# sbi-dev/sbi

Measured on AMD Instinct MI355X. Metric: NPE train (theta,x)-pairs/sec, higher is better.
Workload: dtype f32; 1 GPU; BASELINE configs[1]: NPE + NSF theta-dim 10, x-dim 10, 100000 simulations (90 000-row training split resident in HBM), batch 65536 per GPU, synthetic linear-Gaussian; step = shuffled batch gather (device sampler) + fused NPE training step (pack, loss fwd+bwd, grad all-reduce, clip+Adam); parallelism=dp1, rccl_ranks=1

## Files before the change

sbi_amd/csrc/nsf_train_kernel.h:

```cpp
#pragma once
#include <hip/hip_runtime.h>
#include <stdlib.h>
#include <string.h>
#include "nsf_device.h"
#include "nsf_plan_layout.h"

#define TR_NW 4
#define TR_ROWS 64
#define TR_MAXCH 4
#define TR_GRID_MAX 256
#define TR_SA 68
#define TR_SB 68
#define TR_SLOT(PT) (16 * (PT) + 1)
#define TR_LDK_FAST 50
#ifndef TR_LA
#define TR_LA 2
#endif
#ifndef TR_SPLINE_PRIO
#define TR_SPLINE_PRIO 0
#endif
#ifndef TR_H_SPLIT
#define TR_H_SPLIT 0
#endif
#ifndef TR_PSTASH
#define TR_PSTASH 1
#endif
#ifndef TR_NO_S0
#define TR_NO_S0 1
#endif

struct TrainPlan {
  int SA, SB, SS;
  int o_A0, o_A1, o_B, o_Bs, o_cnt;
  int o_xs;
  int o_wave, w_total;
  int w_zs, w_gys, w_gzs;
  int DCHB, PTW;
  int nch[2];
  int PLP;
  int grid, ntiles;
  int lds_floats;
  int overlay;
  float* grad_x;
};

constexpr int build_train_layout(const NsfPlan& pl, TrainPlan* tp) {
  if (pl.D > 15 || pl.H > 64 || pl.NB > 2 || (pl.NB < 1 && !pl.ctx_mlp)) return SBI_AMD_E_UNSUPPORTED;
  const int d_id_max = pl.shape[0].d_id > pl.shape[1].d_id ? pl.shape[0].d_id : pl.shape[1].d_id;
  if (d_id_max + pl.C + 1 > 32 || pl.C + 1 > 32) return SBI_AMD_E_UNSUPPORTED;
  tp->DCHB = 4 / pl.PT;
  if (tp->DCHB < 1) return SBI_AMD_E_UNSUPPORTED;
  if (tp->DCHB > 2) tp->DCHB = 2;
  tp->PTW = 16 * pl.PT;
  for (int par = 0; par < 2; ++par) {
    tp->nch[par] = (pl.shape[par].d_tr + tp->DCHB - 1) / tp->DCHB;
    if (tp->nch[par] > TR_MAXCH) return SBI_AMD_E_UNSUPPORTED;
  }
  tp->SA = TR_SA;
// ... 44 lines not shown
  if (NSF_DBG_ABL(pl.ablate, 512) && tp->grid > 4) tp->grid = 4;
  return 0;
}

constexpr sbi_amd_nsf_config kNsfDefaultCfg = {10, 10, 50, 10, 5, 2, 3.0f, 1e-3f, 1e-3f, 1e-3f, 1e-3f};
constexpr NsfPlan nsf_make_static_plan() {
  NsfPlan p{};
  nsf_build_layout(&kNsfDefaultCfg, TR_NW, &p);
  return p;
}
constexpr NsfPlan kStaticPl = nsf_make_static_plan();
constexpr TrainPlan nsf_make_static_train() {
  TrainPlan t{};
  build_train_layout(kStaticPl, &t);
  return t;
}
constexpr TrainPlan kStaticTp = nsf_make_static_train();
static_assert(kStaticPl.n_params == 98025 && kStaticTp.overlay == 0 && kStaticTp.nch[0] == 3, "default NSF layout");

static bool plan_is_static_default(const NsfPlan& pl, const TrainPlan& tp) {
  NsfPlan a = pl;
  a.B = a.min_w = a.min_h = a.min_d = a.lu_eps = a.sqrt_h = a.inv_sqrt_h = 0.f;
  a.one_minus_kw = a.one_minus_kh = a.d_const = a.log_z = 0.f;
  a.ablate = 0;
  const NsfPlan b = kStaticPl;
  if (memcmp(&a, &b, sizeof(NsfPlan)) != 0) return false;
  TrainPlan c = tp;
  c.grid = c.ntiles = 0;
  c.grad_x = nullptr;
  const TrainPlan d = kStaticTp;
  return memcmp(&c, &d, sizeof(TrainPlan)) == 0 && NSF_DBG_ABL(pl.ablate, 0x40000) == 0;
}

__device__ __forceinline__ void stage_D(float* __restrict__ st, int SA, int row, const LaneId& id,
                                        const f4 (&v)[NSF_HT], bool relu) {
#pragma unroll
  for (int mt = 0; mt < NSF_HT; ++mt)
#pragma unroll
    for (int r = 0; r < 4; ++r) {
      float a = v[mt][r];
      st[row * SA + 16 * mt + 4 * r + id.g] = relu ? fmaxf(a, 0.f) : a;
    }
}

__device__ __forceinline__ int il_col(int c) { return 4 * (c & 15) + (c >> 4); }
__device__ __forceinline__ void stage_DB(float* __restrict__ st, int SB, int row, const LaneId& id,
                                         const f4 (&v)[NSF_HT], bool relu) {
  static_assert(NSF_HT == 4, "one float4 per register row");
#pragma unroll
  for (int r = 0; r < 4; ++r) {
    f4 w = {v[0][r], v[1][r], v[2][r], v[3][r]};
    if (relu) w = {fmaxf(w[0], 0.f), fmaxf(w[1], 0.f), fmaxf(w[2], 0.f), fmaxf(w[3], 0.f)};
    *(f4*)(st + row * SB + 4 * (4 * r + id.g)) = w;
  }
}

__device__ __forceinline__ constexpr int dw_krow(int s) { return 16 * (s >> 2) + (s & 3); }

template <int NT, int SA, int SB, bool IL = false>
__device__ __forceinline__ void dw_gemm(const float* __restrict__ Ast, const float* __restrict__ Bst,
                                        int acol0, int bcol0, const LaneId& id, f4 (&acc)[NT], int nt_on = NT,
                                        int abl = 0, f4* accb = nullptr) {
  if (abl & 1) return;
  const float ones_b = id.j == 0 ? 1.f : 0.f;
  constexpr int KS = TR_ROWS / 4, LA = NT >= 3 ? TR_LA : 2 * TR_LA;
  const float* ap = Ast + 4 * id.g * SA + acol0 + id.j;
  const float* bp = IL ? Bst + 4 * id.g * SB + 4 * id.j + (bcol0 >> 4) : Bst + 4 * id.g * SB + bcol0 + id.j;
  float a[LA + 1], b[LA + 1][NT];
  auto load_b = [&](int u, int s) {
    if (IL && NT == 4) {
      const f4 w = *(const f4*)(bp + dw_krow(s) * SB);
#pragma unroll
      for (int nt = 0; nt < NT; ++nt) b[u][nt] = w[nt];
    } else {
#pragma unroll
      for (int nt = 0; nt < NT; ++nt) b[u][nt] = bp[dw_krow(s) * SB + (IL ? nt : 16 * nt)];
    }
  };
#pragma unroll
  for (int u = 0; u < LA; ++u) {
    a[u] = ap[dw_krow(u) * SA];
    load_b(u, u);
  }
#pragma unroll
  for (int s = 0; s < KS; ++s) {
    if (s + LA < KS) {
      a[(s + LA) % (LA + 1)] = ap[dw_krow(s + LA) * SA];
      load_b((s + LA) % (LA + 1), s + LA);
    }
    __builtin_amdgcn_sched_barrier(0);
#pragma unroll
    for (int nt = 0; nt < NT; ++nt)
      if (NT == 1 || nt < nt_on) acc[nt] = MFMA16(a[s % (LA + 1)], b[s % (LA + 1)][nt], acc[nt]);
    if (accb) *accb = MFMA16(a[s % (LA + 1)], ones_b, *accb);
    __builtin_amdgcn_sched_barrier(0);
  }
}

template <int NT, int SA>
__device__ __forceinline__ void dw_gemm_rs(const float* __restrict__ Ast, const float* __restrict__ Bst, int SBr,
                                           int acol0, int bcol0, const LaneId& id, f4 (&acc)[NT], int nt_on = NT,
                                           int abl = 0) {
  if (abl & 1) return;
  constexpr int KS = TR_ROWS / 4, LA = NT >= 4 ? TR_LA : 2 * TR_LA;
  const float* ap = Ast + 4 * id.g * SA + acol0 + id.j;
  const float* bp = Bst + 4 * id.g * SBr + bcol0 + id.j;
  float a[LA + 1], b[LA + 1][NT];
#pragma unroll
  for (int u = 0; u < LA; ++u) {
    a[u] = ap[dw_krow(u) * SA];
#pragma unroll
    for (int nt = 0; nt < NT; ++nt) b[u][nt] = bp[dw_krow(u) * SBr + 16 * nt];
  }
#pragma unroll
  for (int s = 0; s < KS; ++s) {
    if (s + LA < KS) {
      a[(s + LA) % (LA + 1)] = ap[dw_krow(s + LA) * SA];
#pragma unroll
      for (int nt = 0; nt < NT; ++nt) b[(s + LA) % (LA + 1)][nt] = bp[dw_krow(s + LA) * SBr + 16 * nt];
    }
    __builtin_amdgcn_sched_barrier(0);
#pragma unroll
    for (int nt = 0; nt < NT; ++nt)
      if (NT == 1 || nt < nt_on) acc[nt] = MFMA16(a[s % (LA + 1)], b[s % (LA + 1)][nt], acc[nt]);
    __builtin_amdgcn_sched_barrier(0);
  }
}

#define MFMA4(a, b, c) __builtin_amdgcn_mfma_f32_4x4x1f32((a), (b), (c), 0, 0, 0)
constexpr int TR_THIN_C0 = 48;
static_assert(kStaticPl.H == TR_THIN_C0 + 2 && kStaticPl.KSH == 13 && kStaticPl.NB == 2,
              "thin remainder: the static layout's hidden width leaves 2 real features (+ bias column) in tile 3");

template <int SA, int SB>
__device__ __forceinline__ void dw_thin(const float* __restrict__ Ast, const float* __restrict__ Bst, const LaneId& id,
                                        f4& accM, f4& accN) {
  const int l = id.lane;
  const float* aM = Ast + TR_THIN_C0 + (l & 3);
  const float* aN = Ast + l;
  const float* bM = Bst + il_col(l);
  const float* bN = Bst + il_col(TR_THIN_C0 + (l & 3));
  constexpr int KS = TR_ROWS / 4;
  float v[2][4][4];
  auto load = [&](int u, int s) {
#pragma unroll
    for (int g = 0; g < 4; ++g) {
      const int r = dw_krow(s) + 4 * g;
      v[u][g][0] = aM[r * SA];
      v[u][g][1] = bM[r * SB];
      v[u][g][2] = aN[r * SA];
      v[u][g][3] = bN[r * SB];
    }
  };
  load(0, 0);
#pragma unroll
  for (int s = 0; s < KS; ++s) {
    if (s + 1 < KS) load((s + 1) & 1, s + 1);
    __builtin_amdgcn_sched_barrier(0);
#pragma unroll
    for (int g = 0; g < 4; ++g) {
      accM = MFMA4(v[s & 1][g][0], v[s & 1][g][1], accM);
      accN = MFMA4(v[s & 1][g][2], v[s & 1][g][3], accN);
    }
    __builtin_amdgcn_sched_barrier(0);
  }
}
template <bool THIN>
__device__ __forceinline__ void dw_hidden(const float* __restrict__ Ast, const float* __restrict__ Bst, int gw,
                                          const LaneId& id, f4 (&acc)[4], int abl) {
  if constexpr (THIN) {
    if (abl & 1) return;
    if (gw == TR_NW - 1) dw_thin<TR_SA, TR_SB>(Ast, Bst, id, acc[0], acc[1]);
    else dw_gemm<3, TR_SA, TR_SB, true>(Ast, Bst, 16 * gw, 0, id, *reinterpret_cast<f4(*)[3]>(&acc[0]));
  } else {
    dw_gemm<4, TR_SA, TR_SB, true>(Ast, Bst, 16 * gw, 0, id, acc, 4, abl, nullptr);
  }
}

__device__ __forceinline__ void load_D(const float* __restrict__ st, int SA, int row, const LaneId& id,
                                       f4 (&v)[NSF_HT]) {
#pragma unroll
  for (int mt = 0; mt < NSF_HT; ++mt)
#pragma unroll
    for (int r = 0; r < 4; ++r) v[mt][r] = st[row * SA + 16 * mt + 4 * r + id.g];
}

__device__ __forceinline__ void grad_wave_sync(int* cnt, int target, int lane) {
  __builtin_amdgcn_fence(__ATOMIC_RELEASE, "workgroup");
  if (lane == 0) __hip_atomic_fetch_add(cnt, 1, __ATOMIC_RELAXED, __HIP_MEMORY_SCOPE_WORKGROUP);
  while (__hip_atomic_load(cnt, __ATOMIC_RELAXED, __HIP_MEMORY_SCOPE_WORKGROUP) < target) __builtin_amdgcn_s_sleep(1);
  __builtin_amdgcn_fence(__ATOMIC_ACQUIRE, "workgroup");
}

template <int KS, int MT, int LDK>
__device__ __forceinline__ void gemm_T_breg_ldk(const float* __restrict__ lds, const LinDesc& L, const LaneId& id,
                                                const f4 (&gb)[NSF_HT], f4 (&acc)[MT]) {
  const int ldk = LDK ? LDK : L.ldk;
  const float* base[MT];
#pragma unroll
  for (int mt = 0; mt < MT; ++mt) {
    const int f = 16 * mt + id.iperm;
    base[mt] = lds + L.l_w + id.g * ldk + (f < L.in ? f : 0);
  }
  const int kstride = 4 * ldk;
  constexpr int NP = (KS + 1) / 2;
  float a[2][2][MT];
#pragma unroll
  for (int u = 0; u < 2; ++u)
#pragma unroll
    for (int mt = 0; mt < MT; ++mt) a[0][u][mt] = u < KS ? base[mt][u * kstride] : 0.f;
#pragma unroll
  for (int p = 0; p < NP; ++p) {
    if (p + 1 < NP) {
#pragma unroll
      for (int u = 0; u < 2; ++u)
#pragma unroll
        for (int mt = 0; mt < MT; ++mt)
// ... 249 lines not shown
      }
#pragma unroll
      for (int p = 0; p < NP; ++p) {
        if (p + 1 < NP) {
#pragma unroll
          for (int u = 0; u < 2; ++u) {
            bb[(p + 1) & 1][u] = brow[4 * (2 * p + 2 + u)];
#pragma unroll
            for (int mt = 0; mt < NSF_HT; ++mt) a[(p + 1) & 1][u][mt] = wcol[mt][(2 * p + 2 + u) * kstride];
          }
        }
        __builtin_amdgcn_sched_barrier(0);
#pragma unroll
        for (int u = 0; u < 2; ++u)
#pragma unroll
          for (int mt = 0; mt < NSF_HT; ++mt) gh[mt] = MFMA16(a[p & 1][u][mt], bb[p & 1][u], gh[mt]);
        __builtin_amdgcn_sched_barrier(0);
      }
    }
  }
#pragma unroll
  for (int mt = 0; mt < NSF_HT; ++mt)
#pragma unroll
    for (int r = 0; r < 4; ++r) gh[mt][r] = (16 * mt + 4 * r + id.g < LF.in) ? gh[mt][r] : 0.f;
}
template <int PT>
__device__ __forceinline__ void wft_chunk(const float* __restrict__ lds, const LinDesc& LF, const NsfPlan& pl,
                                          const ShapeDesc& S, const LaneId& id, const float* __restrict__ Arow,
                                          int SA, int d0, f4 (&gh)[NSF_HT]) {
  if (LF.ldk == TR_LDK_FAST) wft_chunk_ldk<PT, TR_LDK_FAST>(lds, LF, pl, S, id, Arow, SA, d0, gh);
  else wft_chunk_ldk<PT, 0>(lds, LF, pl, S, id, Arow, SA, d0, gh);
}

__device__ __forceinline__ void write_tile(float* __restrict__ part, const LinDesc& L, int out0, int nt,
                                           const LaneId& id, const f4& acc) {
#pragma unroll
  for (int r = 0; r < 4; ++r) {
    const int out = out0 + 4 * id.g + r;
    const int in = 16 * nt + id.j;
    if (out < L.out) {
      if (in < L.in) part[L.g_w + out * L.in + in] = acc[r];
      else if (in == L.in) part[L.g_b + out] = acc[r];
    }
  }
}
__device__ __forceinline__ void write_thin(float* __restrict__ part, const LinDesc& L, const LaneId& id, const f4& accM,
                                           const f4& accN) {
  const int l = id.lane;
#pragma unroll
  for (int m = 0; m < 4; ++m) {
    const int outM = TR_THIN_C0 + m, inM = l;
    if (outM < L.out) {
      if (inM < L.in) part[L.g_w + outM * L.in + inM] = accM[m];
      else if (inM == L.in) part[L.g_b + outM] = accM[m];
    }
    const int outN = 4 * (l >> 2) + m, inN = TR_THIN_C0 + (l & 3);
    if (l < TR_THIN_C0 && outN < L.out) {
      if (inN < L.in) part[L.g_w + outN * L.in + inN] = accN[m];
      else if (inN == L.in) part[L.g_b + outN] = accN[m];
    }
  }
}
__device__ __forceinline__ void write_bias(float* __restrict__ part, const LinDesc& L, int out0, const LaneId& id,
                                           const f4& accb) {
  if (id.j != 0) return;
#pragma unroll
  for (int r = 0; r < 4; ++r) {
    const int out = out0 + 4 * id.g + r;
    if (out < L.out) part[L.g_b + out] = accb[r];
  }
}

__device__ __forceinline__ constexpr int cm_reps(const NsfPlan& pl) { return pl.ctx_reps; }
struct BwdIo {
  int t_hi, t_lo;
  const float* packed;
  const float* zstats;
  const float* stash;
  const float* x;
  const float* noise;
  float* gz[2];
  const float* row_w;
  float uni_w;
  long long n, x_rows;
  float* partial;
  float* grad_theta;
  const float* astash;
  const float* pstash;
  long long* dbg;
};
template <int K, int KSH, int NBT, int NCH, int NTW, bool HB, int SP = 0>
__global__ void __launch_bounds__(128 * TR_NW, HB ? 1 : 2)
nsf_bwd_layer_kernel(const NsfPlan pl_, const TrainPlan tp_, const BwdIo io) {
// ... 2 lines not shown
  const float* __restrict__ x = io.x;
  const float* __restrict__ row_w = io.row_w;
  const float uni_w = io.uni_w;
  const long long n = io.n, x_rows = io.x_rows;
  float* __restrict__ partial = io.partial;
  float* __restrict__ grad_theta = io.grad_theta;
  const float* __restrict__ astash = io.astash;
  long long* __restrict__ dbg = io.dbg;
  const NsfPlan& pl = SP != 0 ? kStaticPl : pl_;
  const TrainPlan& tp = SP != 0 ? kStaticTp : tp_;
#ifdef NSF_DEBUG
  const int dbg_tile_sel = pl_.ablate & 128;
#define NSF_ABL(bit) (pl_.ablate & (bit))
#define NSF_ABLV (pl_.ablate)
#define TS(i) do { if (dbg && t == 0 && blockIdx.x == 0 && (threadIdx.x & 63) == 0 && tile == (int)(blockIdx.x + (dbg_tile_sel ? gridDim.x : 0))) \
    dbg[(threadIdx.x >> 6) * 64 + (i)] = (long long)__builtin_readcyclecounter(); } while (0)
#else
#define NSF_ABL(bit) 0
#define NSF_ABLV 0
#define TS(i) do { } while (0)
#endif
  constexpr int PT = (3 * K - 1 + 15) / 16;
  constexpr int DCHB = (4 / PT) > 2 ? 2 : (4 / PT);
  extern __shared__ __attribute__((aligned(16))) float lds[];
  const int tid = threadIdx.x;
  const int wave = tid >> 6;
  const LaneId id = make_lane();
  constexpr bool cm = (NBT == 0);
  constexpr int NB = cm ? 1 : NBT;
  const int SLOTS = nsf_ast_slots(pl);
  const int reps = cm_reps(pl);
  const int D = pl.D, C = pl.C;
  constexpr int SA = TR_SA, SB = TR_SB;
  const int SS = tp.SS;
  float* Bt = lds + tp.o_B;
  float* Bs = lds + tp.o_Bs;
  const float* x_mean = zstats + 2 * D;
  const float* x_std = x_mean + C;

  if (NSF_ABL(256)) {
    for (int i = tid; i < tp.lds_floats; i += blockDim.x) lds[i] = __builtin_nanf("");
    __syncthreads();
  }
  const bool ov = tp.overlay != 0;
  if (!ov) stage_layer(lds, packed + (long long)io.t_hi * pl.img_floats, pl.lds_w_train_floats, tid, blockDim.x);
  if (tid == 0) *(int*)(lds + tp.o_cnt) = 0;
  if (tid < 32) {
    lds[tp.o_xs + tid] = tid < C ? x_mean[tid] : 0.f;
    lds[tp.o_xs + 32 + tid] = tid < C ? 1.f / x_std[tid] : 1.f;
  }
  const float* xs = lds + tp.o_xs;
  const int ntc = (C + 1 + 15) / 16;
  const f4 zero4 = {0.f, 0.f, 0.f, 0.f};
  const bool multi = (int)(blockIdx.x + gridDim.x) < tp_.ntiles;
#define BWD_T_VARS                                                                                                  \
  const int par = cm ? 0 : (t & 1);                                                                                 \
  const ShapeDesc& S = pl.shape[(SP != 0 || cm) ? 0 : par];                                                         \
  const bool is_last = (t == pl.T - 1);                                                                             \
  const float* img = packed + (long long)t * pl.img_floats;                                                         \
  const int F0 = ov ? S.final_off : 0;                                                                              \
  const float* ldsF = lds - F0;                                                                                     \
  const LinDesc& L0 = S.lin[0];                                                                                     \
  const LinDesc& LF = S.lin[S.fin];                                                                                 \
  const int nch = tp.nch[(SP != 0 || cm) ? 0 : par];                                                                \
  const int nt0 = (S.in0 + 1 + 15) / 16;                               \
                     \
// ... 4 lines not shown
  if (wave < TR_NW) {
    float* sc = lds + tp.o_wave + wave * tp.w_total;
    float* zs = sc + tp.w_zs;
    float* gys = sc + tp.w_gys;
    float* gzs = sc + tp.w_gzs;
    const int arow0 = 16 * wave;
    for (int i = id.lane; i < tp.w_total; i += 64) sc[i] = 0.f;
    const LaneId id0 = id;
    float zv[4], gv[4], xv[8], wv;
    auto fetch_inputs = [&](int t_, int tile_, const LaneId& id) {
      const long long row_ = (long long)tile_ * TR_ROWS + arow0 + id.j;
      const long long rs = row_ < n ? row_ : 0;
      const long long xr = (x_rows == n) ? rs : (x_rows == 1 ? 0 : rs % x_rows);
      const float* z_in = io.stash + (long long)t_ * n * D;
      const float* gz_up = (t_ == pl.T - 1) ? io.noise : io.gz[(t_ + 1) & 1];
      const int d_id_ = pl.shape[(SP != 0 || cm) ? 0 : (t_ & 1)].d_id;
#pragma unroll
      for (int u = 0; u < 4; ++u) {
        const int d = id.g + 4 * u;
        const int dc = d < D ? d : 0;
        zv[u] = z_in[rs * D + dc];
        gv[u] = __hip_atomic_load(gz_up + rs * D + dc, __ATOMIC_RELAXED, __HIP_MEMORY_SCOPE_AGENT);
      }
#pragma unroll
      for (int u = 0; u < 8; ++u) {
        const int c = id.g + 4 * u - d_id_;
        xv[u] = x[xr * C + ((c >= 0 && c < C) ? c : 0)];
      }
      wv = row_w ? row_w[rs] : uni_w;
    };
    for (int t = io.t_hi; t >= io.t_lo; --t) {
    BWD_T_VARS
    LaneId id = id0;
    asm volatile("" : "+v"(id.lane), "+v"(id.j), "+v"(id.g), "+v"(id.iperm));
    float* __restrict__ gz_dn = io.gz[t & 1];
    if (t == io.t_hi || !multi) fetch_inputs(t, blockIdx.x, id);
    for (int tile = blockIdx.x; tile < tp_.ntiles; tile += gridDim.x) {
      LaneId id = id0;
      asm volatile("" : "+v"(id.j), "+v"(id.g), "+v"(id.iperm));
      const long long row = (long long)tile * TR_ROWS + arow0 + id.j;
      const bool valid = row < n;
      const float wn = valid ? wv : 0.f;
      const float gld = -wn;
      const int trow = arow0 + id.j;
      const bool need_s0 = !TR_NO_S0 || ov || tile == (int)blockIdx.x;
      if (need_s0) __syncthreads();
      if (ov) {
        stage_layer(lds, img + F0, pl.lds_w_train_floats - F0, tid, blockDim.x);
        __syncthreads();
      }
      TS(0);
      float gzr[4];
      {
#pragma unroll
        for (int u = 0; u < 4; ++u) {
          const int d = id.g + 4 * u;
          const float gz = (valid && d < D) ? gv[u] : 0.f;
          gzr[u] = is_last ? wn * gz : gz;
          if (d < D) {
            zs[id.j * pl.ZW + d] = valid ? zv[u] : 0.f;
            gzs[id.j * pl.ZW + d] = gzr[u];
          }
        }
        wave_lds_fence();
#pragma unroll
        for (int u = 0; u < 8; ++u) {
          const int k = id.g + 4 * u;
          const int c = k - S.d_id;
          const int cc = (c >= 0 && c < C) ? c : 0;
          const int zd = 2 * k + (1 - par);
          const float zid = zs[id.j * pl.ZW + (zd < D ? zd : 0)];
          const float ctx = ((valid ? xv[u] : 0.f) - xs[cc]) * xs[32 + cc];
          float v = (k == S.in0) ? 1.f : 0.f;
          v = (c >= 0 && c < C) ? ctx : v;
          v = (k < S.d_id) ? zid : v;
          if (k < SS) Bs[trow * SS + k] = v;
        }
        for (int k = 32 + id.g; k < SS; k += 4) Bs[trow * SS + k] = 0.f;
      }
      float gus_r[4] = {0.f, 0.f, 0.f, 0.f};
      if (cm) {
        for (int k = id.g; k < D; k += 4) gys[id.j * pl.ZW + k] = gzs[id.j * pl.ZW + k];
      } else if (!(NSF_ABL(64))) {
        const float* Lm = ldsF + S.l_L;
        const float* Um = ldsF + S.l_U;
        f4 gu = zero4, gy = zero4;
        float al[4], bz[4], au[4];
#pragma unroll
        for (int s4 = 0; s4 < 4; ++s4) {
          al[s4] = Lm[(4 * s4 + id.g) * 16 + id.j];
          bz[s4] = gzr[s4];
          au[s4] = Um[(4 * id.g + s4) * 16 + id.j];
        }
#pragma unroll
        for (int s4 = 0; s4 < 4; ++s4) gu = MFMA16(al[s4], bz[s4], gu);
#pragma unroll
        for (int s4 = 0; s4 < 4; ++s4) gy = MFMA16(au[s4], gu[s4], gy);
#pragma unroll
        for (int ii = 0; ii < 4; ++ii) {
          gus_r[ii] = gu[ii];
          if (4 * id.g + ii < D) gys[id.j * pl.ZW + 4 * id.g + ii] = gy[ii];
        }
      }
      wave_lds_fence();
      const long long nt16 = (n + 15) / 16;
      const long long wt16 = (long long)tile * TR_NW + wave < nt16 ? (long long)tile * TR_NW + wave : nt16 - 1;
      const float* ast = astash + (((long long)t * nt16 + wt16) * SLOTS) * 1024 +
                         4 * id.lane;
      TS(1);
      __syncthreads();
      TS(2);

      f4 bt1[NSF_HT], bt2[NSF_HT], bsg[NSF_HT];
      f4 hpre[cm ? 2 : 1][NSF_HT];
      if (TR_SPLINE_PRIO) __builtin_amdgcn_s_setprio(TR_SPLINE_PRIO);
      for (int c = 0; c < nch; ++c) {
        const int d0 = c * DCHB;
        const int slot = id.g & 1, part = id.g >> 1;
        const int dd = d0 + slot;
        float* pp = lds + ((c & 1) ? tp.o_A1 : tp.o_A0) + trow * SA + slot * TR_SLOT(PT);
        if (slot < DCHB) {
          if (dd < S.d_tr && !(NSF_ABL(4))) {
            const int zi = id.j * pl.ZW + 2 * dd + par;
            float yv, gxv;
            rq_spline_pair_bwd<K>(pp, tp.PTW, zs[zi], gys[zi], gld, pl_, part, yv, gxv);
            if (part == 0) {
              zs[zi] = yv;
              gys[zi] = gxv;
            }
          } else if (part == 0) {
            for (int k = 0; k < tp.PTW; ++k) pp[k] = 0.f;
          }
        }
        TS(3 + c);
        __syncthreads();
      }
      if (TR_SPLINE_PRIO) __builtin_amdgcn_s_setprio(0);
      if (cm) {
        ast_load<KSH>(ast, reps > 0 ? reps - 1 : 0, hpre[0]);
        if (reps > 0) ast_load<KSH>(ast, reps, hpre[1]);
      } else {
        ast_load<KSH>(ast, 2 + 4 * (NB - 1), bt2);
        ast_load<KSH>(ast, 3 + 4 * (NB - 1), bsg);
        ast_load<KSH>(ast, 1 + 4 * (NB - 1), bt1);
      }
      float us_r[4] = {0.f, 0.f, 0.f, 0.f};
      if (!cm && !(NSF_ABL(64))) {
        const float* Um = ldsF + S.l_U;
        float au[4], by[4];
#pragma unroll
        for (int s4 = 0; s4 < 4; ++s4) {
          au[s4] = Um[id.j * 16 + 4 * s4 + id.g];
          by[s4] = zs[id.j * pl.ZW + 4 * s4 + id.g];
        }
        f4 uv = zero4;
#pragma unroll
        for (int s4 = 0; s4 < 4; ++s4) uv = MFMA16(au[s4], by[s4], uv);
#pragma unroll
        for (int ii = 0; ii < 4; ++ii) us_r[ii] = uv[ii];
      }
      {
        const int nxt = tile + (int)gridDim.x;
        const bool more = nxt < tp_.ntiles, hop = !more && multi && t > io.t_lo;
        fetch_inputs(hop ? t - 1 : t, more ? nxt : (hop ? (int)blockIdx.x : tile), id);
      }
      TS(8);
      __syncthreads();
      if (ov) {
        stage_layer(lds, img, S.final_off, tid, blockDim.x);
        __syncthreads();
      }
      TS(9);
      const bool hsplit = TR_H_SPLIT && !cm && !ov;
      f4 gh[NSF_HT];
      load_D(lds + o_AX, SA, trow, id, gh);
      wave_lds_fence();
      const bool want_gx = tp_.grad_x != nullptr;
      float* gx_row = want_gx ? tp_.grad_x + (valid ? row : 0) * C : nullptr;

      if (cm) {
        f4 ga[NSF_HT], gb[NSF_HT];
        for (int i = reps; i >= 1; --i) {
          if (i < reps) {
            ast_load<KSH>(ast, i - 1, hpre[0]);
            ast_load<KSH>(ast, i, hpre[1]);
            __syncthreads();
          }
#pragma unroll
          for (int mt = 0; mt < NSF_HT; ++mt)
#pragma unroll
            for (int r = 0; r < 4; ++r) ga[mt][r] = hpre[1][mt][r] > 0.f ? gh[mt][r] : 0.f;
          stage_D(lds + o_AY, SA, trow, id, ga, false);
          stage_DB(Bt, SB, trow, id, hpre[0], true);
          if (!HB && id.g == 0) Bt[trow * SB + il_col(pl.H)] = 1.f;
          __syncthreads();
#pragma unroll
          for (int mt = 0; mt < NSF_HT; ++mt) gb[mt] = zero4;
          gemm_T_breg<KSH, NSF_HT>(lds, S.lin[1], id, ga, gb, NSF_ABLV);
#pragma unroll
          for (int mt = 0; mt < NSF_HT; ++mt) gh[mt] = gb[mt];
        }
#pragma unroll
        for (int mt = 0; mt < NSF_HT; ++mt)
#pragma unroll
          for (int r = 0; r < 4; ++r) gh[mt][r] = hpre[0][mt][r] > 0.f ? gh[mt][r] : 0.f;
      } else {
#pragma unroll
        for (int b = NB - 1; b >= 0; --b) {
          f4 ga[NSF_HT], gb[NSF_HT];
          {
            f4 gc[NSF_HT];
#pragma unroll
            for (int mt = 0; mt < NSF_HT; ++mt)
#pragma unroll
              for (int r = 0; r < 4; ++r) {
                const float sgm = bsg[mt][r];
                ga[mt][r] = gh[mt][r] * sgm;
                gc[mt][r] = gh[mt][r] * bt2[mt][r] * sgm * (1.f - sgm);
              }
            stage_D(lds + o_AX, SA, trow, id, gc, false);
            if (want_gx)
              ctx_grad_update<KSH>(lds, S.lin[1 + 3 * b], id, gc, 0, C, xs, gx_row, valid, is_last && b == NB - 1);
            if (hsplit && b == NB - 1) {
              TS(50);
              __syncthreads();
              TS(51);
            }
            stage_D(lds + o_AY, SA, trow, id, ga, false);
          }
          stage_DB(Bt, SB, trow, id, bt1, true);
          if (!HB && id.g == 0) Bt[trow * SB + il_col(pl.H)] = 1.f;
          ast_load<KSH>(ast, 4 * b, hpre[0]);
          if (b > 0) {
            ast_load<KSH>(ast, 2 + 4 * (b - 1), bt2);
            ast_load<KSH>(ast, 3 + 4 * (b - 1), bsg);
          }
          TS(20 + 8 * b);
          __syncthreads();
          TS(21 + 8 * b);
#pragma unroll
          for (int mt = 0; mt < NSF_HT; ++mt) gb[mt] = zero4;
          gemm_T_breg<KSH, NSF_HT>(lds, S.lin[3 + 3 * b], id, ga, gb, NSF_ABLV);
#pragma unroll
          for (int mt = 0; mt < NSF_HT; ++mt)
#pragma unroll
            for (int r = 0; r < 4; ++r) ga[mt][r] = bt1[mt][r] > 0.f ? gb[mt][r] : 0.f;
          if (b > 0) ast_load<KSH>(ast, 1 + 4 * (b - 1), bt1);
          TS(22 + 8 * b);
          __syncthreads();
          TS(23 + 8 * b);
          stage_D(lds + o_AY, SA, trow, id, ga, false);
          stage_DB(Bt, SB, trow, id, hpre[0], true);
          if (!HB && id.g == 0) Bt[trow * SB + il_col(pl.H)] = 1.f;
          __syncthreads();
          TS(24 + 8 * b);
#pragma unroll
          for (int mt = 0; mt < NSF_HT; ++mt) gb[mt] = zero4;
          gemm_T_breg<KSH, NSF_HT>(lds, S.lin[2 + 3 * b], id, ga, gb, NSF_ABLV);
#pragma unroll
          for (int mt = 0; mt < NSF_HT; ++mt)
#pragma unroll
            for (int r = 0; r < 4; ++r) gh[mt][r] += hpre[0][mt][r] > 0.f ? gb[mt][r] : 0.f;
          TS(25 + 8 * b);
          if (b > 0) __syncthreads();
        }
      }

      stage_D(lds + o_AX, SA, trow, id, gh, false);
      TS(40);
      __syncthreads();
      TS(41);
      {
        f4 gin[1];
        gin[0] = zero4;
        gemm_T_breg<KSH, 1>(lds, L0, id, gh, gin, NSF_ABLV);
#pragma unroll
        for (int r = 0; r < 4; ++r) {
          const int k = 4 * r + id.g;
          if (k < S.d_id) gys[id.j * pl.ZW + 2 * k + (1 - par)] += gin[0][r];
        }
      }
      if (want_gx) ctx_grad_update<KSH>(lds, L0, id, gh, S.d_id, C, xs, gx_row, valid, is_last && cm);
      if (!cm) {
        float* Ay = lds + o_AY + trow * SA;
#pragma unroll
        for (int ii = 0; ii < 4; ++ii) {
          const int k = 4 * id.g + ii;
          const int o = id.j * pl.ZW + k;
          Ay[k] = k < D ? gus_r[ii] : (k == D ? gld : 0.f);
          Ay[16 + k] = k < D ? gzs[o] : 0.f;
          Bt[trow * SB + il_col(k)] = k < D ? zs[o] : (k == D ? 1.f : 0.f);
          Bt[trow * SB + il_col(16 + k)] = k < D ? us_r[ii] : (k == D ? 1.f : 0.f);
        }
      }
      TS(42);
      __syncthreads();
      for (int d = id.g; d < D; d += 4) {
        if (valid) {
          const float g = gys[id.j * pl.ZW + d];
          if (t > 0) gz_dn[row * D + d] = g;
          else if (grad_theta) grad_theta[row * D + d] = g * zstats[D + d];
        }
      }
      TS(43);
    }
    if (t > io.t_lo && !ov) stage_layer(lds, packed + (long long)(t - 1) * pl.img_floats, pl.lds_w_train_floats, tid, 64 * TR_NW);
    }

  } else {
    const int gw = wave - TR_NW;
    int* cnt = (int*)(lds + tp.o_cnt);
    int sync_target = 0;
    const LaneId id0 = id;
    f4 hl[NSF_HT];
    auto fetch_hl = [&](int t_, int tile_) {
      const long long nt16 = (n + 15) / 16;
      const long long wt16 = (long long)tile_ * TR_NW + gw < nt16 ? (long long)tile_ * TR_NW + gw : nt16 - 1;
      const float* ast = astash + (((long long)t_ * nt16 + wt16) * SLOTS) * 1024 +
                         4 * id0.lane;
      ast_load<KSH>(ast, cm ? reps : 4 * NB, hl);
    };
    constexpr bool use_pst = TR_PSTASH != 0;
    f4 pq[DCHB][PT];
    auto pq_load = [&](int t_, int tile_, int c_) {
      const long long nt16 = (n + 15) / 16;
      const long long wt16 = (long long)tile_ * TR_NW + gw < nt16 ? (long long)tile_ * TR_NW + gw : nt16 - 1;
      const float* pstw = io.pstash + ((long long)t_ * nt16 + wt16) * nsf_pst_tile_floats(pl) + 4 * id0.lane;
      const int d_tr_ = pl.shape[(SP != 0 || cm) ? 0 : (t_ & 1)].d_tr;
#pragma unroll
      for (int sl = 0; sl < DCHB; ++sl) {
        const int dd = c_ * DCHB + sl;
#pragma unroll
        for (int pt = 0; pt < PT; ++pt) pq[sl][pt] = pst_load<PT>(pstw, dd < d_tr_ ? dd : d_tr_ - 1, pt);
      }
    };
    auto pq_store = [&](float* __restrict__ arow, const LaneId& id, int c_, int d_tr_) {
#pragma unroll
      for (int sl = 0; sl < DCHB; ++sl)
        if (c_ * DCHB + sl < d_tr_) {
#pragma unroll
          for (int pt = 0; pt < PT; ++pt)
#pragma unroll
            for (int r = 0; r < 4; ++r) arow[id.j * SA + sl * TR_SLOT(PT) + 16 * pt + 4 * r + id.g] = pq[sl][pt][r];
        }
    };
    fetch_hl(io.t_hi, blockIdx.x);
    if (use_pst) pq_load(io.t_hi, blockIdx.x, 0);
    for (int t = io.t_hi; t >= io.t_lo; --t) {
    BWD_T_VARS
    LaneId id = id0;
    asm volatile("" : "+v"(id.lane), "+v"(id.j), "+v"(id.g), "+v"(id.iperm));
    f4 acc0[NTW], accC[NB][NTW], acc1[NB][4], acc2[NB][4], accF[NCH][4], accLU[1];
    f4 acc1b[HB ? NB : 1], acc2b[HB ? NB : 1], accFb[HB ? NCH : 1];
  #pragma unroll
    for (int i = 0; i < (HB ? NB : 1); ++i) { acc1b[i] = zero4; acc2b[i] = zero4; }
  #pragma unroll
    for (int i = 0; i < (HB ? NCH : 1); ++i) accFb[i] = zero4;
  #pragma unroll
    for (int i = 0; i < NTW; ++i) acc0[i] = zero4;
  #pragma unroll
    for (int b = 0; b < NB; ++b) {
  #pragma unroll
      for (int i = 0; i < NTW; ++i) accC[b][i] = zero4;
  #pragma unroll
      for (int i = 0; i < 4; ++i) { acc1[b][i] = zero4; acc2[b][i] = zero4; }
    }
  #pragma unroll
    for (int c = 0; c < NCH; ++c)
  #pragma unroll
      for (int i = 0; i < 4; ++i) accF[c][i] = zero4;
    accLU[0] = zero4;

    for (int tile = blockIdx.x; tile < tp_.ntiles; tile += gridDim.x) {
      LaneId id = id0;
      asm volatile("" : "+v"(id.j), "+v"(id.g), "+v"(id.iperm));
      const int trow = 16 * gw + id.j;
      const bool more_tiles = tile + (int)gridDim.x < tp_.ntiles;
      const int t_nxt = more_tiles ? t : (t > io.t_lo ? t - 1 : t);
      const int tile_nxt = more_tiles ? tile + (int)gridDim.x : (t > io.t_lo ? (int)blockIdx.x : tile);
      const bool need_s0 = !TR_NO_S0 || ov || tile == (int)blockIdx.x;
      if (need_s0) __syncthreads();
      else { sync_target += 4; grad_wave_sync(cnt, sync_target, id.lane); }
      if (ov) {
        stage_layer(lds, img + F0, pl.lds_w_train_floats - F0, tid, blockDim.x);
        __syncthreads();
      }
      TS(0);
      stage_DB(Bt, SB, trow, id, hl, false);
      if (!HB && id.g == 0) Bt[trow * SB + il_col(pl.H)] = 1.f;
      if (use_pst) {
        pq_store(lds + tp.o_A0 + 16 * gw * SA, id, 0, S.d_tr);
        if (1 < nch) pq_load(t, tile, 1);
      } else if (!(NSF_ABL(32))) final_layer_chunk_T<PT, KSH>(ldsF, lds + tp.o_A0 + 16 * gw * SA, pl, tp, S, id, hl, 0);
      f4 gh[NSF_HT];
  #pragma unroll
      for (int mt = 0; mt < NSF_HT; ++mt) gh[mt] = zero4;
      TS(1);
      __syncthreads();
      TS(2);
  #pragma unroll
      for (int k = 0; k <= NCH; ++k) {
        if (k <= nch) {
          if (k >= 1) {
            const int oa = ((k - 1) & 1) ? tp.o_A1 : tp.o_A0;
            const bool hsplit = TR_H_SPLIT && !cm && !ov;
            if (hsplit && k == nch) {
              if (!(NSF_ABL(2))) wft_chunk<PT>(ldsF, LF, pl, S, id, lds + oa + 16 * gw * SA, SA, (k - 1) * DCHB, gh);
              stage_D(lds + o_AX, SA, trow, id, gh, false);
              TS(9);
              __syncthreads();
            }
            if (!HB && DCHB == 2 && k == nch && (S.d_tr & 1)) {
              f4 (&af)[4] = accF[k - 1 < NCH ? k - 1 : 0];
              f4 part[PT < 3 ? PT : 1];
#pragma unroll
              for (int i = 0; i < (PT < 3 ? PT : 1); ++i) part[i] = af[i];
              dw_gemm<(PT < 3 ? PT : 1), TR_SA, TR_SB, true>(lds + oa, Bt, 16 * (gw % PT), 16 * PT * (gw / PT), id, part,
                                                             PT < 3 ? PT : 1, NSF_ABLV, nullptr);
#pragma unroll
              for (int i = 0; i < (PT < 3 ? PT : 1); ++i) af[i] = part[i];
            } else
            dw_gemm<4, TR_SA, TR_SB, true>(lds + oa, Bt, 16 * gw + (gw / PT < DCHB ? gw / PT : 0), 0, id,
                                           accF[k - 1 < NCH ? k - 1 : 0], 4, NSF_ABLV,
                                           HB ? &accFb[k - 1 < NCH ? k - 1 : 0] : nullptr);
            TS(13 + k);
            if (!(hsplit && k == nch) && !(NSF_ABL(2)))
              wft_chunk<PT>(ldsF, LF, pl, S, id, lds + oa + 16 * gw * SA, SA, (k - 1) * DCHB, gh);
          }
          TS(3 + 2 * k);
          if (k + 1 < nch) {
            if (k >= 1) { sync_target += 4; grad_wave_sync(cnt, sync_target, id.lane); }
            TS(17 + k);
            if (use_pst) {
              pq_store(lds + (((k + 1) & 1) ? tp.o_A1 : tp.o_A0) + 16 * gw * SA, id, k + 1, S.d_tr);
              if (k + 2 < nch) pq_load(t, tile, k + 2);
            } else if (!(NSF_ABL(32)))
              final_layer_chunk_T<PT, KSH>(ldsF, lds + (((k + 1) & 1) ? tp.o_A1 : tp.o_A0) + 16 * gw * SA, pl, tp, S, id,
                                           hl, (k + 1) * DCHB);
          }
          if (k == nch && !(TR_H_SPLIT && !cm && !ov)) stage_D(lds + o_AX, SA, trow, id, gh, false);
          TS(4 + 2 * k);
          __syncthreads();
          if (ov && k == nch) {
            stage_layer(lds, img, S.final_off, tid, blockDim.x);
            __syncthreads();
          }
        }
      }
      if (cm) {
        for (int i = reps; i >= 1; --i) {
          if (i < reps) __syncthreads();
          __syncthreads();
          dw_gemm<4, TR_SA, TR_SB, true>(lds + o_AY, Bt, 16 * gw, 0, id, acc1[0], 4, NSF_ABLV, HB ? &acc1b[0] : nullptr);
        }
      } else {
  #pragma unroll
        for (int b = NB - 1; b >= 0; --b) {
          __syncthreads();
          TS(21 + 8 * b);
          if constexpr (SP != 0) dw_hidden<true>(lds + o_AY, Bt, gw, id, acc2[b], NSF_ABLV);
          else dw_gemm<4, TR_SA, TR_SB, true>(lds + o_AY, Bt, 16 * gw, 0, id, acc2[b], 4, NSF_ABLV, HB ? &acc2b[b] : nullptr);
          TS(22 + 8 * b);
          __syncthreads();
          dw_gemm_rs<NTW, TR_SA>(lds + o_AX, Bs, SS, 16 * gw, S.d_id, id, accC[b], ntc, NSF_ABLV);
          __syncthreads();
          TS(24 + 8 * b);
          if constexpr (SP != 0) dw_hidden<true>(lds + o_AY, Bt, gw, id, acc1[b], NSF_ABLV);
          else dw_gemm<4, TR_SA, TR_SB, true>(lds + o_AY, Bt, 16 * gw, 0, id, acc1[b], 4, NSF_ABLV, HB ? &acc1b[b] : nullptr);
          TS(25 + 8 * b);
          if (b > 0) __syncthreads();
        }
      }
      __syncthreads();
      TS(41);
      fetch_hl(t_nxt, tile_nxt);
      if (use_pst) pq_load(t_nxt, tile_nxt, 0);
      dw_gemm_rs<NTW, TR_SA>(lds + o_AX, Bs, SS, 16 * gw, 0, id, acc0, nt0, NSF_ABLV);
      TS(42);
      __syncthreads();
      if (gw < 2 && !cm) dw_gemm<1, TR_SA, TR_SB, true>(lds + o_AY, Bt, 16 * gw, 16 * gw, id, accLU);
      TS(43);
    }

    float* part = partial + ((long long)t * gridDim.x + blockIdx.x) * tp.PLP;
    const int out0 = 16 * gw;
  #pragma unroll
    for (int nt = 0; nt < NTW; ++nt) write_tile(part, L0, out0, nt, id, acc0[nt]);
    if (cm) {
  #pragma unroll
      for (int nt = 0; nt < 4; ++nt) write_tile(part, S.lin[1], out0, nt, id, acc1[0][nt]);
      if (HB) write_bias(part, S.lin[1], out0, id, acc1b[0]);
    } else {
  #pragma unroll
      for (int b = 0; b < NB; ++b) {
  #pragma unroll
        for (int nt = 0; nt < NTW; ++nt) write_tile(part, S.lin[1 + 3 * b], out0, nt, id, accC[b][nt]);
        if (SP != 0 && gw == TR_NW - 1) {
          write_thin(part, S.lin[2 + 3 * b], id, acc1[b][0], acc1[b][1]);
          write_thin(part, S.lin[3 + 3 * b], id, acc2[b][0], acc2[b][1]);
        } else {
  #pragma unroll
          for (int nt = 0; nt < (SP != 0 ? 3 : 4); ++nt) {
            write_tile(part, S.lin[2 + 3 * b], out0, nt, id, acc1[b][nt]);
            write_tile(part, S.lin[3 + 3 * b], out0, nt, id, acc2[b][nt]);
          }
        }
        if (HB) {
          write_bias(part, S.lin[2 + 3 * b], out0, id, acc1b[b]);
          write_bias(part, S.lin[3 + 3 * b], out0, id, acc2b[b]);
        }
      }
    }
  #pragma unroll
    for (int c = 0; c < NCH; ++c) {
      if (c < nch) {
        if (!HB && DCHB == 2 && c == nch - 1 && (S.d_tr & 1)) {
          const int dd = c * DCHB, pt = gw % PT;
  #pragma unroll
          for (int i = 0; i < (PT < 3 ? PT : 1); ++i)
  #pragma unroll
            for (int r = 0; r < 4; ++r) {
              const int p = 16 * pt + 4 * id.g + r;
              const int in = 16 * (PT * (gw / PT) + i) + id.j;
              if (p < pl.P) {
                const int out = dd * pl.P + p;
                if (in < LF.in) part[LF.g_w + out * LF.in + in] = accF[c][i][r];
                else if (in == LF.in) part[LF.g_b + out] = accF[c][i][r];
              }
            }
          continue;
        }
        const int dd = c * DCHB + gw / PT;
        const int pt = gw % PT;
        if (gw < DCHB * PT && dd < S.d_tr) {
  #pragma unroll
          for (int nt = 0; nt < 4; ++nt)
  #pragma unroll
            for (int r = 0; r < 4; ++r) {
              const int p = 16 * pt + 4 * id.g + r;
              const int in = 16 * nt + id.j;
              if (p < pl.P) {
                const int out = dd * pl.P + p;
                if (in < LF.in) part[LF.g_w + out * LF.in + in] = accF[c][nt][r];
                else if (in == LF.in) part[LF.g_b + out] = accF[c][nt][r];
                if (HB && nt == 0 && id.j == 0) part[LF.g_b + out] = accFb[c][r];
              }
            }
        }
      }
    }
    if (!cm) {
      const int ntri = D * (D - 1) / 2;
      float* plow = part + S.g_lu;
      float* pup = plow + ntri;
      float* pdiag = pup + ntri;
      float* pbias = pdiag + D;
  #pragma unroll
      for (int r = 0; r < 4; ++r) {
        const int i = 4 * id.g + r, k = id.j;
        const float v = accLU[0][r];
        if (gw == 0) {
          if (i < D && k < D) {
            if (k > i) pup[i * D - i * (i + 1) / 2 + (k - i - 1)] = v;
            else if (k == i) pdiag[i] = v;
          } else if (i == D && k == D) part[S.n_params] = v;
        } else if (gw == 1) {
          if (i < D) {
            if (k < i) plow[i * (i - 1) / 2 + k] = v;
            else if (k == D) pbias[i] = v;
          }
        }
      }
    }
    }

  }
#undef BWD_T_VARS
// ... 80 lines not shown
```

Measured before the change: 92.08 million pairs/s.

## Store staged gradient tiles in a float4-friendly permuted column layout

Adds an AF layout mode, on when SP != 0, in which stage_D and load_D move whole f4 rows instead of four scalar strided LDS accesses. The weight-gradient GEMMs compensate by reading A with a permuted lane column (id.iperm), and the thin remainder path remaps its columns through fo_col. Partial-gradient writeout is folded into a single branchless write_entry with a select-computed offset, and optional ISA phase markers are added. This is meant to cut LDS instruction count and bank traffic on the backward staging path. It depends on iperm and fo_col matching the new layout exactly in every consumer.

```diff
diff --git a/sbi_amd/csrc/nsf_train_kernel.h b/sbi_amd/csrc/nsf_train_kernel.h
--- a/sbi_amd/csrc/nsf_train_kernel.h
+++ b/sbi_amd/csrc/nsf_train_kernel.h
@@ -24,6 +24,11 @@
 #endif
 #ifndef TR_PSTASH
 #define TR_PSTASH 1
+#endif
+#ifdef NSF_ISA_MARKS
+#define TR_MARK(name) asm volatile("; @phase " name)
+#else
+#define TR_MARK(name) do { } while (0)
 #endif
 #ifndef TR_NO_S0
 #define TR_NO_S0 1
@@ -134,15 +139,24 @@
   return memcmp(&c, &d, sizeof(TrainPlan)) == 0 && NSF_DBG_ABL(pl.ablate, 0x40000) == 0;
 }
 
+__device__ __forceinline__ constexpr int fo_col(int c) { return (c & ~15) + 4 * (c & 3) + ((c >> 2) & 3); }
+template <bool AF>
 __device__ __forceinline__ void stage_D(float* __restrict__ st, int SA, int row, const LaneId& id,
                                         const f4 (&v)[NSF_HT], bool relu) {
 #pragma unroll
-  for (int mt = 0; mt < NSF_HT; ++mt)
-#pragma unroll
-    for (int r = 0; r < 4; ++r) {
-      float a = v[mt][r];
-      st[row * SA + 16 * mt + 4 * r + id.g] = relu ? fmaxf(a, 0.f) : a;
-    }
+  for (int mt = 0; mt < NSF_HT; ++mt) {
+    if constexpr (AF) {
+      f4 w = v[mt];
+      if (relu) w = {fmaxf(w[0], 0.f), fmaxf(w[1], 0.f), fmaxf(w[2], 0.f), fmaxf(w[3], 0.f)};
+      *(f4*)(st + row * SA + 16 * mt + 4 * id.g) = w;
+    } else {
+#pragma unroll
+      for (int r = 0; r < 4; ++r) {
+        float a = v[mt][r];
+        st[row * SA + 16 * mt + 4 * r + id.g] = relu ? fmaxf(a, 0.f) : a;
+      }
+    }
+  }
 }
 
 __device__ __forceinline__ int il_col(int c) { return 4 * (c & 15) + (c >> 4); }
@@ -159,14 +173,14 @@
 
 __device__ __forceinline__ constexpr int dw_krow(int s) { return 16 * (s >> 2) + (s & 3); }
 
-template <int NT, int SA, int SB, bool IL = false>
+template <int NT, int SA, int SB, bool IL = false, bool AF = false>
 __device__ __forceinline__ void dw_gemm(const float* __restrict__ Ast, const float* __restrict__ Bst,
                                         int acol0, int bcol0, const LaneId& id, f4 (&acc)[NT], int nt_on = NT,
                                         int abl = 0, f4* accb = nullptr) {
   if (abl & 1) return;
   const float ones_b = id.j == 0 ? 1.f : 0.f;
   constexpr int KS = TR_ROWS / 4, LA = NT >= 3 ? TR_LA : 2 * TR_LA;
-  const float* ap = Ast + 4 * id.g * SA + acol0 + id.j;
+  const float* ap = Ast + 4 * id.g * SA + acol0 + (AF ? id.iperm : id.j);
   const float* bp = IL ? Bst + 4 * id.g * SB + 4 * id.j + (bcol0 >> 4) : Bst + 4 * id.g * SB + bcol0 + id.j;
   float a[LA + 1], b[LA + 1][NT];
   auto load_b = [&](int u, int s) {
@@ -199,13 +213,13 @@
   }
 }
 
-template <int NT, int SA>
+template <int NT, int SA, bool AF>
 __device__ __forceinline__ void dw_gemm_rs(const float* __restrict__ Ast, const float* __restrict__ Bst, int SBr,
                                            int acol0, int bcol0, const LaneId& id, f4 (&acc)[NT], int nt_on = NT,
                                            int abl = 0) {
   if (abl & 1) return;
   constexpr int KS = TR_ROWS / 4, LA = NT >= 4 ? TR_LA : 2 * TR_LA;
-  const float* ap = Ast + 4 * id.g * SA + acol0 + id.j;
+  const float* ap = Ast + 4 * id.g * SA + acol0 + (AF ? id.iperm : id.j);
   const float* bp = Bst + 4 * id.g * SBr + bcol0 + id.j;
   float a[LA + 1], b[LA + 1][NT];
 #pragma unroll
@@ -238,8 +252,8 @@
 __device__ __forceinline__ void dw_thin(const float* __restrict__ Ast, const float* __restrict__ Bst, const LaneId& id,
                                         f4& accM, f4& accN) {
   const int l = id.lane;
-  const float* aM = Ast + TR_THIN_C0 + (l & 3);
-  const float* aN = Ast + l;
+  const float* aM = Ast + fo_col(TR_THIN_C0 + (l & 3));
+  const float* aN = Ast + fo_col(l);
   const float* bM = Bst + il_col(l);
   const float* bN = Bst + il_col(TR_THIN_C0 + (l & 3));
   constexpr int KS = TR_ROWS / 4;
@@ -273,18 +287,24 @@
   if constexpr (THIN) {
     if (abl & 1) return;
     if (gw == TR_NW - 1) dw_thin<TR_SA, TR_SB>(Ast, Bst, id, acc[0], acc[1]);
-    else dw_gemm<3, TR_SA, TR_SB, true>(Ast, Bst, 16 * gw, 0, id, *reinterpret_cast<f4(*)[3]>(&acc[0]));
+    else dw_gemm<3, TR_SA, TR_SB, true, true>(Ast, Bst, 16 * gw, 0, id, *reinterpret_cast<f4(*)[3]>(&acc[0]));
   } else {
     dw_gemm<4, TR_SA, TR_SB, true>(Ast, Bst, 16 * gw, 0, id, acc, 4, abl, nullptr);
   }
 }
 
+template <bool AF>
 __device__ __forceinline__ void load_D(const float* __restrict__ st, int SA, int row, const LaneId& id,
                                        f4 (&v)[NSF_HT]) {
 #pragma unroll
-  for (int mt = 0; mt < NSF_HT; ++mt)
-#pragma unroll
-    for (int r = 0; r < 4; ++r) v[mt][r] = st[row * SA + 16 * mt + 4 * r + id.g];
+  for (int mt = 0; mt < NSF_HT; ++mt) {
+    if constexpr (AF) {
+      v[mt] = *(const f4*)(st + row * SA + 16 * mt + 4 * id.g);
+    } else {
+#pragma unroll
+      for (int r = 0; r < 4; ++r) v[mt][r] = st[row * SA + 16 * mt + 4 * r + id.g];
+    }
+  }
 }
 
 __device__ __forceinline__ void grad_wave_sync(int* cnt, int target, int lane) {
@@ -600,33 +620,22 @@
   else wft_chunk_ldk<PT, 0>(lds, LF, pl, S, id, Arow, SA, d0, gh);
 }
 
+__device__ __forceinline__ void write_entry(float* __restrict__ part, const LinDesc& L, int out, int in, float v) {
+  const unsigned o = in < L.in ? (unsigned)(L.g_w + out * L.in + in) : (unsigned)(L.g_b + out);
+  if (out < L.out && in <= L.in) part[o] = v;
+}
 __device__ __forceinline__ void write_tile(float* __restrict__ part, const LinDesc& L, int out0, int nt,
                                            const LaneId& id, const f4& acc) {
 #pragma unroll
-  for (int r = 0; r < 4; ++r) {
-    const int out = out0 + 4 * id.g + r;
-    const int in = 16 * nt + id.j;
-    if (out < L.out) {
-      if (in < L.in) part[L.g_w + out * L.in + in] = acc[r];
-      else if (in == L.in) part[L.g_b + out] = acc[r];
-    }
-  }
+  for (int r = 0; r < 4; ++r) write_entry(part, L, out0 + 4 * id.g + r, 16 * nt + id.j, acc[r]);
 }
 __device__ __forceinline__ void write_thin(float* __restrict__ part, const LinDesc& L, const LaneId& id, const f4& accM,
                                            const f4& accN) {
   const int l = id.lane;
 #pragma unroll
   for (int m = 0; m < 4; ++m) {
-    const int outM = TR_THIN_C0 + m, inM = l;
-    if (outM < L.out) {
-      if (inM < L.in) part[L.g_w + outM * L.in + inM] = accM[m];
-      else if (inM == L.in) part[L.g_b + outM] = accM[m];
-    }
-    const int outN = 4 * (l >> 2) + m, inN = TR_THIN_C0 + (l & 3);
-    if (l < TR_THIN_C0 && outN < L.out) {
-      if (inN < L.in) part[L.g_w + outN * L.in + inN] = accN[m];
-      else if (inN == L.in) part[L.g_b + outN] = accN[m];
-    }
+    write_entry(part, L, TR_THIN_C0 + m, l, accM[m]);
+    write_entry(part, L, l < TR_THIN_C0 ? 4 * (l >> 2) + m : L.out, TR_THIN_C0 + (l & 3), accN[m]);
   }
 }
 __device__ __forceinline__ void write_bias(float* __restrict__ part, const LinDesc& L, int out0, const LaneId& id,
@@ -695,6 +704,7 @@
   const int reps = cm_reps(pl);
   const int D = pl.D, C = pl.C;
   constexpr int SA = TR_SA, SB = TR_SB;
+  constexpr bool AF = SP != 0;
   const int SS = tp.SS;
   float* Bt = lds + tp.o_B;
   float* Bs = lds + tp.o_Bs;
@@ -765,6 +775,7 @@
     for (int t = io.t_hi; t >= io.t_lo; --t) {
     BWD_T_VARS
     LaneId id = id0;
+    TR_MARK("row.transform");
     asm volatile("" : "+v"(id.lane), "+v"(id.j), "+v"(id.g), "+v"(id.iperm));
     float* __restrict__ gz_dn = io.gz[t & 1];
     if (t == io.t_hi || !multi) fetch_inputs(t, blockIdx.x, id);
@@ -783,6 +794,7 @@
         __syncthreads();
       }
       TS(0);
+      TR_MARK("row.prologue");
       float gzr[4];
       {
 #pragma unroll
@@ -843,6 +855,7 @@
       TS(1);
       __syncthreads();
       TS(2);
+      TR_MARK("row.spline");
 
       f4 bt1[NSF_HT], bt2[NSF_HT], bsg[NSF_HT];
       f4 hpre[cm ? 2 : 1][NSF_HT];
@@ -868,6 +881,7 @@
         TS(3 + c);
         __syncthreads();
       }
+      TR_MARK("row.gh_handover");
       if (TR_SPLINE_PRIO) __builtin_amdgcn_s_setprio(0);
       if (cm) {
         ast_load<KSH>(ast, reps > 0 ? reps - 1 : 0, hpre[0]);
@@ -904,9 +918,10 @@
         __syncthreads();
       }
       TS(9);
+      TR_MARK("row.blocks");
       const bool hsplit = TR_H_SPLIT && !cm && !ov;
       f4 gh[NSF_HT];
-      load_D(lds + o_AX, SA, trow, id, gh);
+      load_D<AF>(lds + o_AX, SA, trow, id, gh);
       wave_lds_fence();
       const bool want_gx = tp_.grad_x != nullptr;
       float* gx_row = want_gx ? tp_.grad_x + (valid ? row : 0) * C : nullptr;
@@ -923,7 +938,7 @@
           for (int mt = 0; mt < NSF_HT; ++mt)
 #pragma unroll
             for (int r = 0; r < 4; ++r) ga[mt][r] = hpre[1][mt][r] > 0.f ? gh[mt][r] : 0.f;
-          stage_D(lds + o_AY, SA, trow, id, ga, false);
+          stage_D<AF>(lds + o_AY, SA, trow, id, ga, false);
           stage_DB(Bt, SB, trow, id, hpre[0], true);
           if (!HB && id.g == 0) Bt[trow * SB + il_col(pl.H)] = 1.f;
           __syncthreads();
@@ -951,7 +966,7 @@
                 ga[mt][r] = gh[mt][r] * sgm;
                 gc[mt][r] = gh[mt][r] * bt2[mt][r] * sgm * (1.f - sgm);
               }
-            stage_D(lds + o_AX, SA, trow, id, gc, false);
+            stage_D<AF>(lds + o_AX, SA, trow, id, gc, false);
             if (want_gx)
               ctx_grad_update<KSH>(lds, S.lin[1 + 3 * b], id, gc, 0, C, xs, gx_row, valid, is_last && b == NB - 1);
             if (hsplit && b == NB - 1) {
@@ -959,7 +974,7 @@
               __syncthreads();
               TS(51);
             }
-            stage_D(lds + o_AY, SA, trow, id, ga, false);
+            stage_D<AF>(lds + o_AY, SA, trow, id, ga, false);
           }
           stage_DB(Bt, SB, trow, id, bt1, true);
           if (!HB && id.g == 0) Bt[trow * SB + il_col(pl.H)] = 1.f;
@@ -982,7 +997,7 @@
           TS(22 + 8 * b);
           __syncthreads();
           TS(23 + 8 * b);
-          stage_D(lds + o_AY, SA, trow, id, ga, false);
+          stage_D<AF>(lds + o_AY, SA, trow, id, ga, false);
           stage_DB(Bt, SB, trow, id, hpre[0], true);
           if (!HB && id.g == 0) Bt[trow * SB + il_col(pl.H)] = 1.f;
           __syncthreads();
@@ -999,7 +1014,8 @@
         }
       }
 
-      stage_D(lds + o_AX, SA, trow, id, gh, false);
+      stage_D<AF>(lds + o_AX, SA, trow, id, gh, false);
+      TR_MARK("row.initial_lu");
       TS(40);
       __syncthreads();
       TS(41);
@@ -1028,6 +1044,7 @@
       }
       TS(42);
       __syncthreads();
+      TR_MARK("row.gz_out");
       for (int d = id.g; d < D; d += 4) {
         if (valid) {
           const float g = gys[id.j * pl.ZW + d];
@@ -1037,6 +1054,7 @@
       }
       TS(43);
     }
+    TR_MARK("row.next_image");
     if (t > io.t_lo && !ov) stage_layer(lds, packed + (long long)(t - 1) * pl.img_floats, pl.lds_w_train_floats, tid, 64 * TR_NW);
     }
 
@@ -1083,6 +1101,7 @@
     BWD_T_VARS
     LaneId id = id0;
     asm volatile("" : "+v"(id.lane), "+v"(id.j), "+v"(id.g), "+v"(id.iperm));
+    TR_MARK("grad.transform");
     f4 acc0[NTW], accC[NB][NTW], acc1[NB][4], acc2[NB][4], accF[NCH][4], accLU[1];
     f4 acc1b[HB ? NB : 1], acc2b[HB ? NB : 1], accFb[HB ? NCH : 1];
   #pragma unroll
@@ -1119,6 +1138,7 @@
         __syncthreads();
       }
       TS(0);
+      TR_MARK("grad.prologue");
       stage_DB(Bt, SB, trow, id, hl, false);
       if (!HB && id.g == 0) Bt[trow * SB + il_col(pl.H)] = 1.f;
       if (use_pst) {
@@ -1131,6 +1151,7 @@
       TS(1);
       __syncthreads();
       TS(2);
+      TR_MARK("grad.chunks");
   #pragma unroll
       for (int k = 0; k <= NCH; ++k) {
         if (k <= nch) {
@@ -1139,7 +1160,7 @@
             const bool hsplit = TR_H_SPLIT && !cm && !ov;
             if (hsplit && k == nch) {
               if (!(NSF_ABL(2))) wft_chunk<PT>(ldsF, LF, pl, S, id, lds + oa + 16 * gw * SA, SA, (k - 1) * DCHB, gh);
-              stage_D(lds + o_AX, SA, trow, id, gh, false);
+              stage_D<AF>(lds + o_AX, SA, trow, id, gh, false);
               TS(9);
               __syncthreads();
             }
@@ -1171,7 +1192,8 @@
               final_layer_chunk_T<PT, KSH>(ldsF, lds + (((k + 1) & 1) ? tp.o_A1 : tp.o_A0) + 16 * gw * SA, pl, tp, S, id,
                                            hl, (k + 1) * DCHB);
           }
-          if (k == nch && !(TR_H_SPLIT && !cm && !ov)) stage_D(lds + o_AX, SA, trow, id, gh, false);
+          if (k == nch) TR_MARK("grad.gh_handover");
+          if (k == nch && !(TR_H_SPLIT && !cm && !ov)) stage_D<AF>(lds + o_AX, SA, trow, id, gh, false);
           TS(4 + 2 * k);
           __syncthreads();
           if (ov && k == nch) {
@@ -1180,11 +1202,12 @@
           }
         }
       }
+      TR_MARK("grad.blocks");
       if (cm) {
         for (int i = reps; i >= 1; --i) {
           if (i < reps) __syncthreads();
           __syncthreads();
-          dw_gemm<4, TR_SA, TR_SB, true>(lds + o_AY, Bt, 16 * gw, 0, id, acc1[0], 4, NSF_ABLV, HB ? &acc1b[0] : nullptr);
+          dw_gemm<4, TR_SA, TR_SB, true, AF>(lds + o_AY, Bt, 16 * gw, 0, id, acc1[0], 4, NSF_ABLV, HB ? &acc1b[0] : nullptr);
         }
       } else {
   #pragma unroll
@@ -1192,29 +1215,31 @@
           __syncthreads();
           TS(21 + 8 * b);
           if constexpr (SP != 0) dw_hidden<true>(lds + o_AY, Bt, gw, id, acc2[b], NSF_ABLV);
-          else dw_gemm<4, TR_SA, TR_SB, true>(lds + o_AY, Bt, 16 * gw, 0, id, acc2[b], 4, NSF_ABLV, HB ? &acc2b[b] : nullptr);
+          else dw_gemm<4, TR_SA, TR_SB, true, AF>(lds + o_AY, Bt, 16 * gw, 0, id, acc2[b], 4, NSF_ABLV, HB ? &acc2b[b] : nullptr);
           TS(22 + 8 * b);
           __syncthreads();
-          dw_gemm_rs<NTW, TR_SA>(lds + o_AX, Bs, SS, 16 * gw, S.d_id, id, accC[b], ntc, NSF_ABLV);
+          dw_gemm_rs<NTW, TR_SA, AF>(lds + o_AX, Bs, SS, 16 * gw, S.d_id, id, accC[b], ntc, NSF_ABLV);
           __syncthreads();
           TS(24 + 8 * b);
           if constexpr (SP != 0) dw_hidden<true>(lds + o_AY, Bt, gw, id, acc1[b], NSF_ABLV);
-          else dw_gemm<4, TR_SA, TR_SB, true>(lds + o_AY, Bt, 16 * gw, 0, id, acc1[b], 4, NSF_ABLV, HB ? &acc1b[b] : nullptr);
+          else dw_gemm<4, TR_SA, TR_SB, true, AF>(lds + o_AY, Bt, 16 * gw, 0, id, acc1[b], 4, NSF_ABLV, HB ? &acc1b[b] : nullptr);
           TS(25 + 8 * b);
           if (b > 0) __syncthreads();
         }
       }
       __syncthreads();
       TS(41);
+      TR_MARK("grad.initial_lu");
       fetch_hl(t_nxt, tile_nxt);
       if (use_pst) pq_load(t_nxt, tile_nxt, 0);
-      dw_gemm_rs<NTW, TR_SA>(lds + o_AX, Bs, SS, 16 * gw, 0, id, acc0, nt0, NSF_ABLV);
+      dw_gemm_rs<NTW, TR_SA, AF>(lds + o_AX, Bs, SS, 16 * gw, 0, id, acc0, nt0, NSF_ABLV);
       TS(42);
       __syncthreads();
       if (gw < 2 && !cm) dw_gemm<1, TR_SA, TR_SB, true>(lds + o_AY, Bt, 16 * gw, 16 * gw, id, accLU);
       TS(43);
     }
 
+    TR_MARK("grad.writeout");
     float* part = partial + ((long long)t * gridDim.x + blockIdx.x) * tp.PLP;
     const int out0 = 16 * gw;
   #pragma unroll
@@ -1255,11 +1280,7 @@
             for (int r = 0; r < 4; ++r) {
               const int p = 16 * pt + 4 * id.g + r;
               const int in = 16 * (PT * (gw / PT) + i) + id.j;
-              if (p < pl.P) {
-                const int out = dd * pl.P + p;
-                if (in < LF.in) part[LF.g_w + out * LF.in + in] = accF[c][i][r];
-                else if (in == LF.in) part[LF.g_b + out] = accF[c][i][r];
-              }
+              if (p < pl.P) write_entry(part, LF, dd * pl.P + p, in, accF[c][i][r]);
             }
           continue;
         }
@@ -1274,8 +1295,7 @@
               const int in = 16 * nt + id.j;
               if (p < pl.P) {
                 const int out = dd * pl.P + p;
-                if (in < LF.in) part[LF.g_w + out * LF.in + in] = accF[c][nt][r];
-                else if (in == LF.in) part[LF.g_b + out] = accF[c][nt][r];
+                write_entry(part, LF, out, in, accF[c][nt][r]);
                 if (HB && nt == 0 && id.j == 0) part[LF.g_b + out] = accFb[c][r];
               }
             }
```

Result: faster. 93.25 million pairs/s, median of 6 (+1.3%).
